# peterbudai/redux

Measured on AMD Instinct MI355X. Metric: encode MB/s (whole node), per-block bitstream bit-exact, higher is better.
Workload: dtype u32

## Files before the change

### redux_amd/csrc/redux_hip.hip

```cpp
#include "redux_coder.hpp"
#include "redux_any.hpp"
#include "redux_gen.hpp"
#include "redux_encode.hpp"
#include "redux_decode.hpp"
#include "redux_decode_adaptive.hpp"
#include "redux_decode_wave.hpp"
#include "redux_decode_cells.hpp"
#include "redux_pack.hpp"
#include "redux_table.hpp"
#include "redux_coop.hpp"
#include "redux_synth.hpp"
#include "redux_static.hpp"
#include "redux_planes.hpp"
#include "redux_delta.hpp"
#include "redux_hist.hpp"
#include "redux_plane_static.hpp"
#include "redux_segment_static.hpp"
#include "redux_crc.hpp"
#include "redux_store.hpp"

#include "../../include/redux_hip.h"

#include <hip/hip_runtime.h>
#include <algorithm>
// ... 64 lines not shown
    a.out_sizes[blk] = (uint32_t)bo;
    a.status[blk]    = st;
    if (a.in_used)
        a.in_used[blk] = bi;
}

static inline uint64_t align_up(uint64_t v, uint64_t a) { return (v + a - 1) / a * a; }

struct Geometry {
    uint64_t nblocks;
    uint64_t slot_bytes;
    uint32_t slot_cap;
    uint32_t rc_n;
    uint32_t nfreeze;
    bool     u16, fixup;
    bool     any;
    bool     gen;
    uint64_t tree_bytes;
    bool     coop;
    bool     coop_linear;
    uint32_t pair_width;
    uint32_t coop_win;
    uint32_t coop_nwin;
    uint64_t off_rc, off_sizes, off_mode, off_slots, off_trees, off_table, off_seen, off_cstate, off_pairs, total;
};

static int check_params(const redux_params *p)
{
    if (!p)
        return REDUX_INVALID_INPUT;
    const int st = redux_params_check(p->symbol_bits, p->freq_bits, p->code_bits);
    if (st != REDUX_OK)
        return st;
    if (p->symbol_bits > 16)
        return REDUX_UNSUPPORTED;
    return REDUX_OK;
}

static bool is_any(const redux_params *p) { return p->symbol_bits != 8 || p->code_bits > 32; }
static uint64_t gen_updates(const redux_params *p, uint32_t block_size)
{
    const uint64_t nsym    = (uint64_t)block_size * 8 / p->symbol_bits;
    const uint64_t nfreeze = ((1ull << p->freq_bits) - 1) - ((1ull << p->symbol_bits) + 1);
    return nsym < nfreeze ? nsym : nfreeze;
}
static bool gen_decode_cells(const redux_params *p, uint32_t block_size)
// ... 49 lines not shown
    const bool     freezes  = 257ull + n > freq_max;
    const uint64_t bits     = freezes ? n * (p->freq_bits + 2) : n * 9;
    return bits / 8 + 1024;
}

static Geometry geometry(const redux_params *p, uint64_t in_len, uint32_t block_size, bool static_model = false, bool allow_coop = true)
{
    Geometry g;
    memset(&g, 0, sizeof g);
    g.nblocks = in_len == 0 ? 1 : (in_len + block_size - 1) / block_size;
    const uint64_t cap = static_model ? ((uint64_t)block_size + 1) * (p->freq_bits + 2) / 8 + 1024 : slot_cap_for(p, block_size);
    g.slot_cap   = cap > 0xFFFFFF00ull ? 0xFFFFFF00u : (uint32_t)cap;
    g.slot_bytes = align_up((uint64_t)g.slot_cap + 32, 128);
    if (((g.slot_bytes / 128) & 1) == 0)
        g.slot_bytes += 128;
    const uint64_t freq_max = (1ull << p->freq_bits) - 1;
    g.nfreeze = (uint32_t)(freq_max - 257);
    const uint64_t maxlen = in_len < block_size ? in_len : block_size;
    g.rc_n  = (uint32_t)((maxlen < g.nfreeze ? maxlen : g.nfreeze) + 1);
    g.u16   = block_size <= 65536;
    g.fixup = (257ull + (uint64_t)(g.rc_n - 1)) >= (1ull << 17);
    g.rc_n += 32;
    g.any = !static_model && is_any(p);
    if (static_model)
        g.rc_n = 0;
    g.gen = !static_model && is_gen(p, block_size) && 64ull * g.slot_bytes < (1ull << 32);
    if (g.gen) {
        const uint64_t k0      = (1ull << p->symbol_bits) + 1;
        const uint64_t nsym    = maxlen * 8 / p->symbol_bits;
        const uint64_t nfreeze = freq_max - k0;
        g.any     = false;
        g.nfreeze = (uint32_t)(nfreeze < 0xFFFFFFFFull ? nfreeze : 0xFFFFFFFFull);
        g.rc_n    = (uint32_t)((nsym < nfreeze ? nsym : nfreeze) + 1 + 32);
        g.u16     = false;
        g.fixup   = true;
        g.tree_bytes = 0;
    }
    if (g.any) {
        g.rc_n       = 0;
        g.u16        = false;
        g.fixup      = true;
        g.tree_bytes = align_up(((1ull << p->symbol_bits) + 2) * 4, 256);
    }
    g.pair_width = g.u16 ? 64u : 1u;
    const uint64_t lanes_total = g.u16 ? (g.nblocks + 63) / 64 * 64 : g.nblocks;
    g.coop_win  = block_size + 1;
// ... 72 lines not shown

static EncKernel pick_encode_kernel(const Geometry &g, const redux_params *p, bool aligned16, uint32_t block_size)
{
    if (g.gen)
        return p->symbol_bits < 8 ? EncKernel::Gen : EncKernel::GenPair;
    if (g.any)
        return EncKernel::Any;
    bool coop = g.coop;
#ifdef REDUX_AB
    if (getenv("REDUX_ENCODE_KERNEL"))
        coop = false;
#endif
    if (coop)
        return p->code_bits == 32 ? EncKernel::CoopCb32 : EncKernel::Coop;
    bool pair = g.u16 && aligned16 && encode_lanes(g, block_size) == 64;
#ifdef REDUX_AB
    const char *force = getenv("REDUX_ENCODE_KERNEL");
    if (force && !strcmp(force, "single"))
        pair = false;
#endif
    if (pair)
        return p->code_bits == 32 ? EncKernel::PairCb32 : EncKernel::Pair;
    return g.u16 ? EncKernel::SingleU16 : EncKernel::SingleU32;
}

static DecKernel pick_decode_kernel(const Geometry &g, const redux_params *p, uint64_t nslots = 0, uint32_t block_size = 0, bool table = false)
{
    if (g.gen) {
        if (gen_needs_fixup(p, block_size))
            return DecKernel::CellsFixup;
        return gen_decode_in_workspace(p, nslots ? nslots : ~0ull) ? DecKernel::CellsWorkspace : DecKernel::Cells;
    }
    if (g.any)
        return DecKernel::Any;
    if (cells8_takes(p, block_size, nslots, table))
        return cells8_needs_fixup(p, block_size) ? DecKernel::Cells8Fixup : DecKernel::Cells8;
    bool wave = nslots != 0 && nslots <= kWaveDecMaxBlocks && !(g.u16 && !g.fixup);
#ifdef REDUX_AB
    if (getenv("REDUX_DECODE_KERNEL"))
        wave = false;
#endif
    if (wave)
        return g.fixup ? DecKernel::WaveFixup : DecKernel::Wave;
    bool lock = g.u16 && !g.fixup;
#ifdef REDUX_AB
    if (getenv("REDUX_DECODE_KERNEL"))
// ... 282 lines not shown
{
    if (check_params(p) != REDUX_OK || block_size == 0)
        return 0;
    return geometry(p, block_size, block_size).slot_cap;
}

uint64_t redux_encode_bound(const redux_params *p, uint64_t in_len, uint32_t block_size)
{
    if (check_params(p) != REDUX_OK || block_size == 0)
        return 0;
    const Geometry g = geometry(p, in_len, block_size);
    return g.nblocks * (uint64_t)g.slot_cap;
}

uint64_t redux_encode_workspace_bytes(const redux_params *p, uint64_t in_len, uint32_t block_size)
{
    if (check_params(p) != REDUX_OK || block_size == 0)
        return 0;
    return geometry(p, in_len, block_size).total;
}

static int encode_slots_impl(const redux_params *p, const void *d_in, uint64_t in_len, uint32_t block_size,
                             const redux_block *d_table, uint64_t tbl_blocks, bool tbl_aligned16, void *d_block_status,
                             void *d_workspace, uint64_t workspace_bytes, void *stream, uint64_t nblocks_real = 0)
{
    int st = check_params(p);
    if (st != REDUX_OK)
        return st;
    if (block_size == 0 || !d_workspace || !d_block_status || (in_len && !d_in))
        return REDUX_INVALID_INPUT;
    const Geometry g = geometry_ws(p, d_table ? tbl_blocks * (uint64_t)block_size : in_len, block_size, workspace_bytes);
    if (d_table && (g.gen || g.any || in_len > 0xFFFFFFFFull || tbl_blocks == 0))
        return tbl_blocks == 0 ? REDUX_INVALID_INPUT : REDUX_UNSUPPORTED;
    if (workspace_bytes < g.total)
        return REDUX_OUTPUT_TOO_SMALL;
    if (((uintptr_t)d_workspace) & 255)
        return REDUX_INVALID_INPUT;
    hipStream_t s  = (hipStream_t)stream;
    uint8_t    *ws = (uint8_t *)d_workspace;

    if (d_table) {
        TableCheckArgs ta;
        ta.in         = d_table;
        ta.out        = (redux_block *)(ws + g.off_table);
        ta.nentries   = tbl_blocks;
        ta.nblocks    = nblocks_real;
        ta.bytes      = in_len;
        ta.block_size = block_size;
// ... 58 lines not shown
    k_fill_rc<<<(g.rc_n + 255) / 256, 256, 0, s>>>((double *)(ws + g.off_rc), g.rc_n);

    EncArgs a;
    a.in         = (const uint8_t *)d_in;
    a.in_len     = in_len;
    a.nblocks    = g.nblocks;
    a.slots      = ws + g.off_slots;
    a.slot_bytes = g.slot_bytes;
    a.sizes      = (uint32_t *)(ws + g.off_sizes);
    a.status     = (int32_t *)d_block_status;
    a.rc         = (const double *)(ws + g.off_rc);
    a.block_size = block_size;
    a.slot_cap   = g.slot_cap;
    a.nfreeze    = g.nfreeze;
    a.code_bits  = p->code_bits;
    a.aligned16  = ((((uintptr_t)d_in) & 15) == 0 && (d_table ? tbl_aligned16 : (block_size & 15) == 0)) ? 1 : 0;
    a.claims     = (uint32_t *)(ws + g.off_mode + 256);
    a.table      = d_table;
    a.pair_width = g.pair_width;
    a.win0 = 0; a.winlen = block_size + 1; a.rc_frozen = 0.0; a.cstate = nullptr; a.cbase = nullptr;
    a.lanes = encode_lanes(g, block_size);
    const uint32_t grid = (uint32_t)((g.nblocks + a.lanes - 1) / a.lanes);
    const EncKernel which = pick_encode_kernel(g, p, a.aligned16 != 0, block_size);
    if (which == EncKernel::PairCb32 || which == EncKernel::Pair || which == EncKernel::CoopCb32 || which == EncKernel::Coop)
        HIP_TRY(hipMemsetAsync(ws + g.off_mode, g.coop_linear ? 2 : (1 | 2), 4, s));
    switch (which) {
    case EncKernel::CoopCb32:
    case EncKernel::Coop: {
        uint2         *pairs = (uint2 *)(ws + g.off_pairs);
        const uint32_t cgrid = (uint32_t)((g.nblocks + 63) / 64);
        const bool     cb32  = which == EncKernel::CoopCb32;
        {
            const double r = 1.0 / (double)(257ull + g.nfreeze);
            uint64_t     u;
            memcpy(&u, &r, 8);
            u += 4;
            memcpy(&a.rc_frozen, &u, 8);
        }
        a.winlen = g.coop_win;
        a.cstate = !g.u16 ? (uint32_t *)(ws + g.off_cstate) : nullptr;
        a.cbase  = a.cstate ? a.cstate + g.nblocks * 8 : nullptr;
        if (g.u16) {
            k_coop_model<false><<<(uint32_t)g.nblocks, 64, 0, s>>>(a, pairs);
            if (g.fixup) {
                if (cb32) k_coop_chain<true, true><<<cgrid, 128, 0, s>>>(a, pairs);
                else      k_coop_chain<false, true><<<cgrid, 128, 0, s>>>(a, pairs);
// ... 34 lines not shown
            }
#undef REDUX_COOP_LAUNCH
        }
        break;
    }
    case EncKernel::PairCb32: k_encode_pair<false, true><<<grid, 128, 0, s>>>(a); break;
    case EncKernel::Pair: k_encode_pair<false, false><<<grid, 128, 0, s>>>(a); break;
    case EncKernel::SingleU16: k_encode<true, false><<<grid, 64, 0, s>>>(a); break;
    case EncKernel::SingleU32: k_encode<false, true><<<grid, 64, 0, s>>>(a); break;
    case EncKernel::Gen:
    case EncKernel::GenPair:
    case EncKernel::Any: break;
    }
    HIP_TRY(hipGetLastError());
    return REDUX_OK;
}

int redux_encode_slots_dev(const redux_params *p, const void *d_in, uint64_t in_len, uint32_t block_size,
                           void *d_block_status, void *d_workspace, uint64_t workspace_bytes, void *stream)
{
    return encode_slots_impl(p, d_in, in_len, block_size, nullptr, 0, false, d_block_status, d_workspace, workspace_bytes, stream);
}

static int compact_with(const Geometry &g, void *d_out, uint64_t out_cap, void *d_out_offsets, void *d_block_status,
                        void *d_summary, void *d_workspace, uint64_t workspace_bytes, void *stream,
                        const redux_block *d_table = nullptr, uint64_t nblocks_real = 0, const uint8_t *d_stored = nullptr,
                        const void *d_raw = nullptr, uint32_t block_size = 0)
{
    if (!d_workspace || !d_block_status || !d_out_offsets || !d_out)
        return REDUX_INVALID_INPUT;
    if (workspace_bytes < g.off_pairs)
        return REDUX_OUTPUT_TOO_SMALL;
    hipStream_t s  = (hipStream_t)stream;
    uint8_t    *ws = (uint8_t *)d_workspace;

    ScanArgs sa;
    sa.sizes   = (const uint32_t *)(ws + g.off_sizes);
    sa.status  = (const int32_t *)d_block_status;
    sa.offsets = (uint64_t *)d_out_offsets;
    sa.summary = (int32_t *)d_summary;
    sa.nblocks = d_table ? nblocks_real : g.nblocks;
    if (scan_is_coalesced(sa))
        k_scan_sizes_coalesced<<<1, 1024, 0, s>>>(sa);
    else
        k_scan_sizes<<<1, 1024, 0, s>>>(sa);

    CompactArgs ca;
    ca.slots      = ws + g.off_slots;
    ca.slot_bytes = g.slot_bytes;
    ca.offsets    = (const uint64_t *)d_out_offsets;
    ca.out        = (uint8_t *)d_out;
    ca.out_cap    = out_cap;
    ca.status     = (int32_t *)d_block_status;
    ca.summary    = (int32_t *)d_summary;
    ca.nblocks    = g.nblocks;
    ca.mode       = (const uint32_t *)(ws + g.off_mode);
    ca.cap_rows   = (uint32_t)(g.slot_bytes / 4);
    ca.table      = d_table;
    ca.stored     = d_stored;
    ca.raw        = (const uint8_t *)d_raw;
    ca.block_size = block_size;
    k_compact<<<(uint32_t)g.nblocks, 256, 0, s>>>(ca);
    if (!g.any && !g.gen && (g.u16 || g.coop)) {
        const uint32_t tiles = (ca.cap_rows + kTileRows - 1) / kTileRows + 1;
        const uint32_t groups = (uint32_t)((g.nblocks + 63) / 64);
        k_compact_rows<<<(groups + 7) / 8 * 8 * tiles, 256, 0, s>>>(ca);
    }
    HIP_TRY(hipGetLastError());
    return REDUX_OK;
}

int redux_compact_slots_dev(const redux_params *p, uint64_t in_len, uint32_t block_size, void *d_out,
                            uint64_t out_cap, void *d_out_offsets, void *d_block_status, void *d_summary,
                            void *d_workspace, uint64_t workspace_bytes, void *stream)
{
    int st = check_params(p);
    if (st != REDUX_OK)
        return st;
    if (block_size == 0)
        return REDUX_INVALID_INPUT;
    return compact_with(geometry_ws(p, in_len, block_size, workspace_bytes), d_out, out_cap, d_out_offsets, d_block_status, d_summary,
                        d_workspace, workspace_bytes, stream);
}

int redux_encode_blocks_dev(const redux_params *p, const void *d_in, uint64_t in_len, uint32_t block_size,
                            void *d_out, uint64_t out_cap, void *d_out_offsets, void *d_block_status,
                            void *d_summary, void *d_workspace, uint64_t workspace_bytes, void *stream)
{
    int st = redux_encode_slots_dev(p, d_in, in_len, block_size, d_block_status, d_workspace, workspace_bytes, stream);
    if (st != REDUX_OK)
        return st;
    return redux_compact_slots_dev(p, in_len, block_size, d_out, out_cap, d_out_offsets, d_block_status, d_summary,
                                   d_workspace, workspace_bytes, stream);
}

int redux_encode_blocks_v_dev(const redux_params *p, const void *d_in, uint64_t in_bytes, const void *d_table,
                              uint64_t nentries, uint64_t nblocks, uint32_t block_size, uint32_t flags, void *d_out,
                              uint64_t out_cap, void *d_out_offsets, void *d_block_status, void *d_summary, void *d_workspace,
                              uint64_t workspace_bytes, void *stream)
{
    if (!d_table || nblocks == 0 || nentries < nblocks)
        return REDUX_INVALID_INPUT;
    if (nentries > 0xFFFFFFF0ull || nblocks > 0xFFFFFFF0ull || !d_block_status || !d_workspace)
        return REDUX_INVALID_INPUT;
    int st = encode_slots_impl(p, d_in, in_bytes, block_size, (const redux_block *)d_table, nentries,
                               (flags & REDUX_V_ALIGNED16) != 0, d_block_status, d_workspace, workspace_bytes, stream, nblocks);
    if (st != REDUX_OK)
        return st;
    const Geometry g = geometry_ws(p, nentries * (uint64_t)block_size, block_size, workspace_bytes);
    st = compact_with(g, d_out, out_cap, d_out_offsets, d_block_status, d_summary, d_workspace, workspace_bytes, stream,
                      (const redux_block *)((uint8_t *)d_workspace + g.off_table), nblocks);
    if (st != REDUX_OK)
        return st;
    k_table_verdict<<<1, 1, 0, (hipStream_t)stream>>>((const uint32_t *)((uint8_t *)d_workspace + g.off_seen) + table_seen_words(nblocks) - 1,
                                                      (int32_t *)d_summary);
    HIP_TRY(hipGetLastError());
    return REDUX_OK;
}

uint64_t redux_block_count_v(const uint64_t *in_len, uint64_t ninputs, uint32_t block_size)
{
    if (block_size == 0 || (ninputs && !in_len))
        return 0;
    uint64_t n = 0;
    for (uint64_t i = 0; i < ninputs; i++)
        n += redux_block_count(in_len[i], block_size);
    return n;
}

uint64_t redux_block_table_v(const uint64_t *in_off, const uint64_t *in_len, uint64_t ninputs, uint32_t block_size,
                             redux_block *table)
{
    const uint64_t nb = redux_block_count_v(in_len, ninputs, block_size);
// ... 559 lines not shown
    HIP_TRY(hipMemsetAsync(ws + g.off_mode, 0, 256, s));
    StaticEncArgs a;
    a.in         = (const uint8_t *)d_in;
    a.in_len     = in_len;
    a.nblocks    = g.nblocks;
    a.slots      = ws + g.off_slots;
    a.slot_bytes = g.slot_bytes;
    a.sizes      = (uint32_t *)(ws + g.off_sizes);
    a.status     = (int32_t *)d_block_status;
    a.rc         = static_rc(cum[kStaticEntries - 1]);
    a.block_size = block_size;
    a.slot_cap   = g.slot_cap;
    a.code_bits  = p->code_bits;
    a.aligned16  = ((((uintptr_t)d_in) & 15) == 0 && (block_size & 15) == 0) ? 1 : 0;
    memcpy(a.tab.cum, cum, sizeof a.tab.cum);
    const uint32_t grid = (uint32_t)((g.nblocks + 63) / 64);
    switch (pick_static_encode_kernel(p, cum[kStaticEntries - 1], g.nblocks)) {
    case StaticEncKernel::Fixup: k_encode_static<true, false><<<grid, 64, 0, s>>>(a); break;
    case StaticEncKernel::Cb32Solo: k_encode_static<false, true, true><<<grid, 64, 0, s>>>(a); break;
    case StaticEncKernel::Cb32: k_encode_static<false, true><<<grid, 64, 0, s>>>(a); break;
    case StaticEncKernel::Narrow: k_encode_static<false, false><<<grid, 64, 0, s>>>(a); break;
    }
    HIP_TRY(hipGetLastError());
    return compact_with(g, d_out, out_cap, d_out_offsets, d_block_status, d_summary, d_workspace, workspace_bytes, stream);
}

int redux_static_decode_blocks_dev(const redux_params *p, const uint32_t *cum, const void *d_in,
                                   const void *d_in_offsets, uint64_t nblocks, uint32_t block_size, void *d_out,
                                   uint64_t out_cap, void *d_out_sizes, void *d_block_status, void *d_summary,
                                   void *stream)
{
    int st = static_check(p, cum);
    if (st != REDUX_OK)
        return st;
    if (block_size == 0 || !d_in_offsets || !d_out_sizes || !d_block_status)
        return REDUX_INVALID_INPUT;
    if (nblocks == 0)
        return REDUX_OK;
    if (out_cap < nblocks * (uint64_t)block_size)
        return REDUX_OUTPUT_TOO_SMALL;
    hipStream_t   s = (hipStream_t)stream;
    StaticDecArgs a;
    a.in         = (const uint8_t *)d_in;
    a.in_offsets = (const uint64_t *)d_in_offsets;
    a.nblocks    = nblocks;
    a.out        = (uint8_t *)d_out;
    a.out_sizes  = (uint32_t *)d_out_sizes;
// ... 624 lines not shown
    a.c.nblocks    = g.nblocks;
    a.c.slots      = ws + g.off_slots;
    a.c.slot_bytes = g.slot_bytes;
    a.c.sizes      = (uint32_t *)(ws + g.off_sizes);
    a.c.status     = (int32_t *)d_block_status;
    a.c.rc         = static_rc(total);
    a.c.block_size = block_size;
    a.c.slot_cap   = g.slot_cap;
    a.c.code_bits  = p->code_bits;
    a.c.aligned16  = ((((uintptr_t)d_x) & 15) == 0 && (block_size & 15) == 0) ? 1 : 0;
    a.t.cum        = (const uint32_t *)d_cum;
    a.t.E          = E;
    a.t.total      = total;
    a.t.rc257      = static_rc(kStaticEntries - 1);
    const uint64_t slots = plane_slots(g.nblocks, E);
    const uint32_t grid  = (uint32_t)(slots * E);
    switch (pick_static_encode_kernel(p, total, 64 * E * slots)) {
    case StaticEncKernel::Fixup: k_encode_plane_static<true, false><<<grid, 64, 0, s>>>(a); break;
    case StaticEncKernel::Cb32Solo: k_encode_plane_static<false, true, true><<<grid, 64, 0, s>>>(a); break;
    case StaticEncKernel::Cb32: k_encode_plane_static<false, true><<<grid, 64, 0, s>>>(a); break;
    case StaticEncKernel::Narrow: k_encode_plane_static<false, false><<<grid, 64, 0, s>>>(a); break;
    }
    HIP_TRY(hipGetLastError());
    return compact_with(g, d_out, out_cap, d_out_offsets, d_block_status, d_summary, d_workspace, workspace_bytes, stream);
}

int redux_plane_static_encode_dev(const redux_params *p, const void *d_cum, uint32_t total, const void *d_in, uint64_t in_len,
                                  uint32_t block_size, uint32_t element_size, void *d_out, uint64_t out_cap, void *d_out_offsets,
                                  void *d_block_status, void *d_summary, void *d_workspace, uint64_t workspace_bytes, void *stream)
{
    int st = plane_static_check(p, element_size, total);
    if (st != REDUX_OK)
        return st;
    if (block_size == 0 || !d_cum || (!d_in && in_len) || !d_block_status || !d_workspace || (((uintptr_t)d_workspace) & 255))
        return REDUX_INVALID_INPUT;
    if (element_size == 1)
        return plane_static_encode_x(p, d_cum, total, d_in, in_len, block_size, 1, d_out, out_cap, d_out_offsets, d_block_status,
                                     d_summary, d_workspace, workspace_bytes, stream);
    const uint64_t copy = planes_copy_bytes(in_len);
    if (workspace_bytes < copy)
        return REDUX_OUTPUT_TOO_SMALL;
    uint8_t *x = (uint8_t *)d_workspace;
    if ((st = redux_planes_dev(d_in, x, in_len, block_size, element_size, 0, stream)) != REDUX_OK)
        return st;
    return plane_static_encode_x(p, d_cum, total, x, in_len, block_size, element_size, d_out, out_cap, d_out_offsets, d_block_status,
                                 d_summary, x + copy, workspace_bytes - copy, stream);
}
// ... 370 lines not shown
    a.c.slots      = ws + g.off_slots;
    a.c.slot_bytes = g.slot_bytes;
    a.c.sizes      = (uint32_t *)(ws + g.off_sizes);
    a.c.status     = (int32_t *)d_block_status;
    a.c.rc         = static_rc(total);
    a.c.block_size = block_size;
    a.c.slot_cap   = g.slot_cap;
    a.c.code_bits  = p->code_bits;
    a.c.aligned16  = ((((uintptr_t)d_x) & 15) == 0 && (block_size & 15) == 0) ? 1 : 0;
    a.t.p.cum      = (const uint32_t *)d_cum;
    a.t.p.E        = E;
    a.t.p.total    = total;
    a.t.p.rc257    = static_rc(kStaticEntries - 1);
    a.t.k          = G / (64 * E);
    const uint64_t slots = plane_slots(g.nblocks, E);
    const uint32_t grid  = (uint32_t)(slots * E);
    switch (pick_static_encode_kernel(p, total, 64 * E * slots)) {
    case StaticEncKernel::Fixup: k_encode_segment_static<true, false><<<grid, 64, 0, s>>>(a); break;
    case StaticEncKernel::Cb32Solo: k_encode_segment_static<false, true, true><<<grid, 64, 0, s>>>(a); break;
    case StaticEncKernel::Cb32: k_encode_segment_static<false, true><<<grid, 64, 0, s>>>(a); break;
    case StaticEncKernel::Narrow: k_encode_segment_static<false, false><<<grid, 64, 0, s>>>(a); break;
    }
    HIP_TRY(hipGetLastError());
    return compact_with(g, d_out, out_cap, d_out_offsets, d_block_status, d_summary, d_workspace, workspace_bytes, stream);
}

int redux_segment_static_encode_dev(const redux_params *p, const void *d_cum, uint32_t total, const void *d_in, uint64_t in_len,
                                    uint32_t block_size, uint32_t element_size, uint32_t segment_blocks, void *d_out, uint64_t out_cap,
                                    void *d_out_offsets, void *d_block_status, void *d_summary, void *d_workspace,
                                    uint64_t workspace_bytes, void *stream)
{
    int st = segment_static_check(p, element_size, segment_blocks, total);
    if (st != REDUX_OK)
        return st;
    if (block_size == 0 || !d_cum || (!d_in && in_len) || !d_block_status || !d_workspace || (((uintptr_t)d_workspace) & 255))
        return REDUX_INVALID_INPUT;
    if (element_size == 1)
        return segment_static_encode_x(p, d_cum, total, d_in, in_len, block_size, 1, segment_blocks, d_out, out_cap, d_out_offsets,
                                       d_block_status, d_summary, d_workspace, workspace_bytes, stream);
    const uint64_t copy = planes_copy_bytes(in_len);
    if (workspace_bytes < copy)
        return REDUX_OUTPUT_TOO_SMALL;
    uint8_t *x = (uint8_t *)d_workspace;
    if ((st = redux_planes_dev(d_in, x, in_len, block_size, element_size, 0, stream)) != REDUX_OK)
        return st;
    return segment_static_encode_x(p, d_cum, total, x, in_len, block_size, element_size, segment_blocks, d_out, out_cap, d_out_offsets,
                                   d_block_status, d_summary, x + copy, workspace_bytes - copy, stream);
// ... 195 lines not shown
}

int redux_encode_stored_dev(const redux_params *p, const void *d_in, uint64_t in_len, uint32_t block_size, uint32_t element_size,
                            uint32_t store_ratio, void *d_out, uint64_t out_cap, void *d_out_offsets, void *d_stored,
                            void *d_block_status, void *d_summary, void *d_workspace, uint64_t workspace_bytes, void *stream)
{
    int st = stored_check(p, block_size, element_size);
    if (st != REDUX_OK)
        return st;
    if (store_ratio > kStoreRatioOne || !d_workspace || !d_stored || !d_block_status || (in_len && !d_in))
        return REDUX_INVALID_INPUT;
    hipStream_t    s    = (hipStream_t)stream;
    const uint64_t copy = element_size > 1 ? planes_copy_bytes(in_len) : 0;
    if (workspace_bytes < copy)
        return REDUX_OUTPUT_TOO_SMALL;
    const void    *x    = d_in;
    if (element_size > 1) {
        if ((st = redux_planes_dev(d_in, d_workspace, in_len, block_size, element_size, 0, stream)) != REDUX_OK)
            return st;
        x = d_workspace;
    }
    uint8_t       *ws  = (uint8_t *)d_workspace + copy;
    const uint64_t wsb = workspace_bytes - copy;
    if ((st = encode_slots_impl(p, x, in_len, block_size, nullptr, 0, false, d_block_status, ws, wsb, stream)) != REDUX_OK)
        return st;
    const Geometry  g = geometry_ws(p, in_len, block_size, wsb);
    StoreSelectArgs sa;
    sa.status     = (const int32_t *)d_block_status;
    sa.sizes      = (uint32_t *)(ws + g.off_sizes);
    sa.stored     = (uint8_t *)d_stored;
    sa.nblocks    = g.nblocks;
    sa.in_len     = in_len;
    sa.block_size = block_size;
    sa.ratio      = store_ratio;
    const uint64_t wgs = (g.nblocks + 255) / 256;
    k_store_select<<<(uint32_t)(wgs < 1024 ? wgs : 1024), 256, 0, s>>>(sa);
    HIP_TRY(hipGetLastError());
    return compact_with(g, d_out, out_cap, d_out_offsets, d_block_status, d_summary, ws, wsb, stream, nullptr, 0,
                        (const uint8_t *)d_stored, x, block_size);
}

int redux_decode_stored_dev(const redux_params *p, const void *d_in, const void *d_in_offsets, const void *d_stored,
                            uint64_t out_len, uint32_t block_size, uint32_t element_size, void *d_out, uint64_t out_cap,
                            void *d_out_sizes, void *d_block_status, void *d_summary, void *d_workspace, uint64_t workspace_bytes,
                            void *stream)
{
    int st = stored_check(p, block_size, element_size);
    if (st != REDUX_OK)
        return st;
    if (!d_workspace || !d_in_offsets || !d_stored || !d_out_sizes || !d_block_status || (out_len && !d_out))
        return REDUX_INVALID_INPUT;
    if (out_cap < out_len || workspace_bytes < redux_decode_stored_workspace_bytes(p, out_len, block_size, element_size))
        return REDUX_OUTPUT_TOO_SMALL;
    if (((uintptr_t)d_workspace) & 255)
        return REDUX_INVALID_INPUT;
    hipStream_t    s       = (hipStream_t)stream;
    const uint64_t nblocks = redux_block_count(out_len, block_size);
    const uint64_t copy    = element_size > 1 ? planes_copy_bytes(nblocks * (uint64_t)block_size) : 0;
    uint8_t       *t       = element_size > 1 ? (uint8_t *)d_workspace : (uint8_t *)d_out;
    redux_block   *table   = (redux_block *)((uint8_t *)d_workspace + copy);
    uint8_t       *dws     = (uint8_t *)table + store_table_bytes(nblocks);
// ... 202 lines not shown
```

### redux_amd/csrc/redux_pack.hpp

```cpp
#pragma once

#include "redux_coder.hpp"
#include "redux_encode.hpp"
#include "redux_store.hpp"

#include "../../include/redux_hip.h"

#include <hip/hip_runtime.h>
#include <stdint.h>

namespace redux {

__global__ void k_summarize(const int32_t *status, uint64_t nblocks, int32_t *summary)
{
    uint32_t bad = 0;
    uint64_t first = ~0ull;
    for (uint64_t b = (uint64_t)blockIdx.x * blockDim.x + threadIdx.x; b < nblocks; b += (uint64_t)gridDim.x * blockDim.x)
        if (status[b] != REDUX_OK) {
            bad++;
            if (first == ~0ull)
                first = b;
        }
    if (bad) {
        atomicAdd(&summary[1], (int32_t)bad);
// ... 187 lines not shown
    if (tid == 0 && a.summary) {
        a.summary[0] = bad_cnt ? (int32_t)(bad_first & 0xFF) : REDUX_OK;
        a.summary[1] = (int32_t)bad_cnt;
    }
}

struct CompactArgs {
    const uint8_t  *slots;
    uint64_t        slot_bytes;
    const uint64_t *offsets;
    uint8_t        *out;
    uint64_t        out_cap;
    int32_t        *status;
    int32_t        *summary;
    uint64_t        nblocks;
    const uint32_t *mode;
    uint32_t        cap_rows;
    const redux_block *table;
    const uint8_t  *stored;
    const uint8_t  *raw;
    uint32_t        block_size;
};

__global__ void __launch_bounds__(256) k_compact(CompactArgs a)
{
    const uint64_t b = blockIdx.x;
    const uint32_t mode = *a.mode;
    if (b >= a.nblocks || ((mode & 1u) && !a.stored))
        return;
    const uint32_t bx  = (mode & 2u) ? 3u : 0u;
    const uint32_t sel = (mode & 2u) ? 0x00010203u : 0x03020100u;
    const uint64_t lb = a.table ? a.table[b].index : b;
    if (lb == kIdleEntry)
        return;
    const bool raw = a.stored && a.stored[lb];
    if ((mode & 1u) && !raw)
        return;
    const uint64_t o0 = a.offsets[lb], o1 = a.offsets[lb + 1];
    const uint32_t tid = threadIdx.x;
    if (o1 > a.out_cap) {
        if (tid == 0) {
            if (a.status[lb] == REDUX_OK)
                a.status[lb] = REDUX_OUTPUT_TOO_SMALL;
            if (a.summary) {
                atomicCAS(&a.summary[0], REDUX_OK, REDUX_OUTPUT_TOO_SMALL);
                atomicAdd(&a.summary[1], 1);
            }
        }
        return;
    }
    const uint32_t n   = (uint32_t)(o1 - o0);
    const uint8_t *src = a.slots + b * a.slot_bytes;
    uint8_t       *dst = a.out + o0;
    if (raw) {
        store_copy(a.raw + lb * a.block_size, dst, n, tid, 256);
        return;
    }

    uint32_t head = (uint32_t)((16 - ((uintptr_t)dst & 15)) & 15);
    if (head > n)
        head = n;
    if (tid < head)
// ... 1 lines not shown
    const uint32_t nchunks = (n - head) >> 4;
    const uint32_t dq = head >> 2, r = head & 3;
    const uint4   *s16 = reinterpret_cast<const uint4 *>(src);
    uint4         *d16 = reinterpret_cast<uint4 *>(dst + head);
    for (uint32_t i = tid; i < nchunks; i += 256) {
        const uint4    A = s16[i], B = s16[i + 1];
        const uint32_t d[8] = {A.x, A.y, A.z, A.w, B.x, B.y, B.z, B.w};
        uint32_t       v[5];
#pragma unroll
        for (int k = 0; k < 5; k++)
            v[k] = __builtin_amdgcn_perm(0u, dq == 0 ? d[k] : dq == 1 ? d[k + 1] : dq == 2 ? d[k + 2] : d[k + 3], sel);
        uint4 o;
        o.x = __builtin_amdgcn_alignbyte(v[1], v[0], r);
        o.y = __builtin_amdgcn_alignbyte(v[2], v[1], r);
        o.z = __builtin_amdgcn_alignbyte(v[3], v[2], r);
        o.w = __builtin_amdgcn_alignbyte(v[4], v[3], r);
        d16[i] = o;
    }
    const uint32_t done = head + (nchunks << 4);
    if (tid < n - done)
        dst[done + tid] = src[(done + tid) ^ bx];
}

constexpr uint32_t kTileRows = 64;
__global__ void __launch_bounds__(256) k_compact_rows(CompactArgs a)
{
    const uint32_t mode = *a.mode;
    if ((mode & 1u) == 0)
        return;
    const uint32_t sel = (mode & 2u) ? 0x00010203u : 0x03020100u;
    __shared__ uint32_t tile[(kTileRows + 1) * 65];
    __shared__ uint64_t s_dst[64];
    __shared__ uint32_t s_n[64], s_sh[64];
    __shared__ uint32_t s_maxj;
    const uint32_t tiles = (a.cap_rows + kTileRows - 1) / kTileRows + 1;
    const uint32_t y   = blockIdx.x >> 3;
    const uint64_t g   = (uint64_t)(y / tiles) * 8 + (blockIdx.x & 7u);
    const uint32_t r0  = (y % tiles) * kTileRows;
    if (g * 64 >= a.nblocks)
        return;
    const uint32_t tid   = threadIdx.x;
    if (tid == 0)
        s_maxj = 0;
    __syncthreads();
    if (tid < 64) {
        const uint64_t b = g * 64 + tid;
        uint64_t       d = 0;
        uint32_t       n = 0, sh = 0;
        const uint64_t lb = b < a.nblocks ? (a.table ? a.table[b].index : b) : kIdleEntry;
        if (lb != kIdleEntry && !(a.stored && a.stored[lb])) {
            const uint64_t o0 = a.offsets[lb], o1 = a.offsets[lb + 1];
            if (o1 <= a.out_cap) {
                n  = (uint32_t)(o1 - o0);
                sh = (uint32_t)((uintptr_t)(a.out + o0) & 3);
                d  = (uint64_t)(uintptr_t)(a.out + o0) - sh;
                atomicMax(&s_maxj, (sh + n + 3) >> 2);
            } else if (r0 == 0) {
                if (a.status[lb] == REDUX_OK)
                    a.status[lb] = REDUX_OUTPUT_TOO_SMALL;
                if (a.summary) {
                    atomicCAS(&a.summary[0], REDUX_OK, REDUX_OUTPUT_TOO_SMALL);
                    atomicAdd(&a.summary[1], 1);
                }
            }
        }
        s_dst[tid] = d;
        s_n[tid]   = n;
        s_sh[tid]  = sh;
    }
    __syncthreads();
    if (r0 >= s_maxj)
        return;
    const uint4 *area = reinterpret_cast<const uint4 *>(a.slots + g * (64 * a.slot_bytes + 128));
    uint4 v[4], lead = make_uint4(0, 0, 0, 0);
#pragma unroll
    for (int q = 0; q < 4; q++) {
        const uint32_t e = tid + 256 * q, r = r0 + (e >> 4);
        v[q] = r < a.cap_rows ? area[(uint64_t)r * 16 + (e & 15)] : make_uint4(0, 0, 0, 0);
    }
    if (tid < 16 && r0 > 0)
        lead = area[(uint64_t)(r0 - 1) * 16 + tid];
#pragma unroll
    for (int q = 0; q < 4; q++) {
        const uint32_t e = tid + 256 * q;
        uint32_t      *w = &tile[((e >> 4) + 1) * 65 + (e & 15) * 4];
        w[0] = v[q].x; w[1] = v[q].y; w[2] = v[q].z; w[3] = v[q].w;
    }
    if (tid < 16) {
        uint32_t *w = &tile[tid * 4];
        w[0] = lead.x; w[1] = lead.y; w[2] = lead.z; w[3] = lead.w;
    }
    __syncthreads();
    const uint32_t wave = tid >> 6, t = tid & 63;
#pragma unroll 2
    for (uint32_t it = 0; it < 4; it++) {
        const uint32_t l  = wave * 16 + it * 4 + (t >> 4);
        const uint32_t jq = (t & 15) * 4;
        const uint64_t d  = s_dst[l];
        const uint32_t n = s_n[l], sh = s_sh[l];
        const uint32_t j0 = r0 + jq;
        if (d == 0 || j0 >= ((sh + n + 3) >> 2))
            continue;
        uint32_t src[5];
#pragma unroll
        for (int c = 0; c < 5; c++)
            src[c] = __builtin_amdgcn_perm(0u, tile[(jq + c) * 65 + l], sel);
        uint32_t w[4];
#pragma unroll
        for (int c = 0; c < 4; c++)
            w[c] = sh ? __builtin_amdgcn_alignbyte(src[c + 1], src[c], 4 - sh) : src[c + 1];
        uint8_t      *A     = reinterpret_cast<uint8_t *>((uintptr_t)d) + 4 * (uint64_t)j0;
        const int64_t first = (int64_t)4 * j0 - sh;
        if (first >= 0 && first + 16 <= (int64_t)n) {
            typedef uint32_t u32x4 __attribute__((ext_vector_type(4), aligned(4)));
            *reinterpret_cast<u32x4 *>(A) = u32x4{w[0], w[1], w[2], w[3]};
        } else {
#pragma unroll
            for (int c = 0; c < 4; c++) {
                const int64_t f = first + 4 * c;
                if (f >= 0 && f + 4 <= (int64_t)n) {
                    *reinterpret_cast<uint32_t *>(A + 4 * c) = w[c];
                } else {
                    for (int i = 0; i < 4; i++)
                        if (f + i >= 0 && f + i < (int64_t)n)
                            A[4 * c + i] = (uint8_t)(w[c] >> (8 * i));
                }
            }
        }
    }
}

}
```

Before: 364,800.

## Make row-compaction persistent with register-prefetched tiles and skip the unused compaction kernel

```diff
diff --git a/redux_amd/csrc/redux_hip.hip b/redux_amd/csrc/redux_hip.hip
--- a/redux_amd/csrc/redux_hip.hip
+++ b/redux_amd/csrc/redux_hip.hip
@@ -110,6 +110,7 @@
     uint32_t pair_width;
     uint32_t coop_win;
     uint32_t coop_nwin;
+    bool     static_model;
     uint64_t off_rc, off_sizes, off_mode, off_slots, off_trees, off_table, off_seen, off_cstate, off_pairs, total;
 };
 
@@ -205,6 +206,7 @@
     g.fixup = (257ull + (uint64_t)(g.rc_n - 1)) >= (1ull << 17);
     g.rc_n += 32;
     g.any = !static_model && is_any(p);
+    g.static_model = static_model;
     if (static_model)
         g.rc_n = 0;
     g.gen = !static_model && is_gen(p, block_size) && 64ull * g.slot_bytes < (1ull << 32);
@@ -323,6 +325,50 @@
     if (pair)
         return p->code_bits == 32 ? EncKernel::PairCb32 : EncKernel::Pair;
     return g.u16 ? EncKernel::SingleU16 : EncKernel::SingleU32;
+}
+
+enum class SlotLayout { Linear, Rows, Either };
+
+static SlotLayout slot_layout_of(EncKernel which, const Geometry &g)
+{
+    switch (which) {
+    case EncKernel::PairCb32:
+    case EncKernel::Pair: return SlotLayout::Rows;
+    case EncKernel::CoopCb32:
+    case EncKernel::Coop: return g.coop_linear ? SlotLayout::Linear : SlotLayout::Rows;
+    default: return SlotLayout::Linear;
+    }
+}
+
+static SlotLayout slot_layout(const Geometry &g, uint32_t block_size)
+{
+    if (g.static_model || g.gen || g.any)
+        return SlotLayout::Linear;
+#ifdef REDUX_AB
+    if (getenv("REDUX_ENCODE_KERNEL"))
+        return SlotLayout::Either;
+#endif
+    if (g.coop)
+        return g.coop_linear ? SlotLayout::Linear : SlotLayout::Rows;
+    if (!g.u16 || encode_lanes(g, block_size) != 64)
+        return SlotLayout::Linear;
+    if (block_size & 15)
+        return SlotLayout::Linear;
+    return SlotLayout::Either;
+}
+
+constexpr uint32_t kCompactRows = 128, kCompactOversub = 2;
+
+template <uint32_t ROWS>
+static void launch_compact_rows(const CompactArgs &ca, uint32_t oversub, bool linear, hipStream_t s)
+{
+    const uint32_t per_cu   = std::min<uint32_t>(8u, (160u << 10) / compact_rows_lds_bytes<ROWS>());
+    const uint32_t resident = cu_count() * per_cu;
+    const uint32_t groups8  = (uint32_t)((ca.nblocks + 63) / 64 + 7) / 8 * 8;
+    const uint32_t tiles    = (ca.cap_rows + ROWS - 1) / ROWS + 1;
+    uint32_t splits = (oversub * resident + groups8 - 1) / groups8;
+    splits = std::max<uint32_t>(1u, std::min<uint32_t>(splits, tiles / kRowsMinTiles));
+    k_compact_rows<ROWS><<<groups8 * splits, 256, 0, s>>>(ca, splits, linear ? 1u : 0u);
 }
 
 static DecKernel pick_decode_kernel(const Geometry &g, const redux_params *p, uint64_t nslots = 0, uint32_t block_size = 0, bool table = false)
@@ -651,8 +697,11 @@
 
 static int encode_slots_impl(const redux_params *p, const void *d_in, uint64_t in_len, uint32_t block_size,
                              const redux_block *d_table, uint64_t tbl_blocks, bool tbl_aligned16, void *d_block_status,
-                             void *d_workspace, uint64_t workspace_bytes, void *stream, uint64_t nblocks_real = 0)
-{
+                             void *d_workspace, uint64_t workspace_bytes, void *stream, uint64_t nblocks_real = 0,
+                             SlotLayout *left = nullptr)
+{
+    if (left)
+        *left = SlotLayout::Linear;
     int st = check_params(p);
     if (st != REDUX_OK)
         return st;
@@ -757,6 +806,8 @@
     a.lanes = encode_lanes(g, block_size);
     const uint32_t grid = (uint32_t)((g.nblocks + a.lanes - 1) / a.lanes);
     const EncKernel which = pick_encode_kernel(g, p, a.aligned16 != 0, block_size);
+    if (left)
+        *left = slot_layout_of(which, g);
     if (which == EncKernel::PairCb32 || which == EncKernel::Pair || which == EncKernel::CoopCb32 || which == EncKernel::Coop)
         HIP_TRY(hipMemsetAsync(ws + g.off_mode, g.coop_linear ? 2 : (1 | 2), 4, s));
     switch (which) {
@@ -837,7 +888,7 @@
     return encode_slots_impl(p, d_in, in_len, block_size, nullptr, 0, false, d_block_status, d_workspace, workspace_bytes, stream);
 }
 
-static int compact_with(const Geometry &g, void *d_out, uint64_t out_cap, void *d_out_offsets, void *d_block_status,
+static int compact_with(const Geometry &g, SlotLayout left, void *d_out, uint64_t out_cap, void *d_out_offsets, void *d_block_status,
                         void *d_summary, void *d_workspace, uint64_t workspace_bytes, void *stream,
                         const redux_block *d_table = nullptr, uint64_t nblocks_real = 0, const uint8_t *d_stored = nullptr,
                         const void *d_raw = nullptr, uint32_t block_size = 0)
@@ -875,11 +926,24 @@
     ca.stored     = d_stored;
     ca.raw        = (const uint8_t *)d_raw;
     ca.block_size = block_size;
-    k_compact<<<(uint32_t)g.nblocks, 256, 0, s>>>(ca);
-    if (!g.any && !g.gen && (g.u16 || g.coop)) {
-        const uint32_t tiles = (ca.cap_rows + kTileRows - 1) / kTileRows + 1;
-        const uint32_t groups = (uint32_t)((g.nblocks + 63) / 64);
-        k_compact_rows<<<(groups + 7) / 8 * 8 * tiles, 256, 0, s>>>(ca);
+    const bool linear_kernel = left == SlotLayout::Linear || d_stored != nullptr;
+    if (linear_kernel)
+        k_compact<<<(uint32_t)g.nblocks, 256, 0, s>>>(ca);
+    if (left != SlotLayout::Linear) {
+        uint32_t rows = kCompactRows, oversub = kCompactOversub;
+#ifdef REDUX_AB
+        if (getenv("REDUX_COMPACT_ROWS"))
+            rows = (uint32_t)atoi(getenv("REDUX_COMPACT_ROWS"));
+        if (getenv("REDUX_COMPACT_OVERSUB"))
+            oversub = (uint32_t)atoi(getenv("REDUX_COMPACT_OVERSUB"));
+        if (rows == 64)
+            launch_compact_rows<64>(ca, oversub, !linear_kernel, s);
+        else if (rows == 256)
+            launch_compact_rows<256>(ca, oversub, !linear_kernel, s);
+        else
+#endif
+        launch_compact_rows<128>(ca, oversub, !linear_kernel, s);
+        (void)rows;
     }
     HIP_TRY(hipGetLastError());
     return REDUX_OK;
@@ -894,19 +958,21 @@
         return st;
     if (block_size == 0)
         return REDUX_INVALID_INPUT;
-    return compact_with(geometry_ws(p, in_len, block_size, workspace_bytes), d_out, out_cap, d_out_offsets, d_block_status, d_summary,
-                        d_workspace, workspace_bytes, stream);
+    const Geometry g = geometry_ws(p, in_len, block_size, workspace_bytes);
+    return compact_with(g, slot_layout(g, block_size), d_out, out_cap, d_out_offsets, d_block_status, d_summary, d_workspace,
+                        workspace_bytes, stream);
 }
 
 int redux_encode_blocks_dev(const redux_params *p, const void *d_in, uint64_t in_len, uint32_t block_size,
                             void *d_out, uint64_t out_cap, void *d_out_offsets, void *d_block_status,
                             void *d_summary, void *d_workspace, uint64_t workspace_bytes, void *stream)
 {
-    int st = redux_encode_slots_dev(p, d_in, in_len, block_size, d_block_status, d_workspace, workspace_bytes, stream);
-    if (st != REDUX_OK)
-        return st;
-    return redux_compact_slots_dev(p, in_len, block_size, d_out, out_cap, d_out_offsets, d_block_status, d_summary,
-                                   d_workspace, workspace_bytes, stream);
+    SlotLayout left;
+    int st = encode_slots_impl(p, d_in, in_len, block_size, nullptr, 0, false, d_block_status, d_workspace, workspace_bytes, stream, 0, &left);
+    if (st != REDUX_OK)
+        return st;
+    return compact_with(geometry_ws(p, in_len, block_size, workspace_bytes), left, d_out, out_cap, d_out_offsets, d_block_status,
+                        d_summary, d_workspace, workspace_bytes, stream);
 }
 
 int redux_encode_blocks_v_dev(const redux_params *p, const void *d_in, uint64_t in_bytes, const void *d_table,
@@ -918,12 +984,13 @@
         return REDUX_INVALID_INPUT;
     if (nentries > 0xFFFFFFF0ull || nblocks > 0xFFFFFFF0ull || !d_block_status || !d_workspace)
         return REDUX_INVALID_INPUT;
+    SlotLayout left;
     int st = encode_slots_impl(p, d_in, in_bytes, block_size, (const redux_block *)d_table, nentries,
-                               (flags & REDUX_V_ALIGNED16) != 0, d_block_status, d_workspace, workspace_bytes, stream, nblocks);
+                               (flags & REDUX_V_ALIGNED16) != 0, d_block_status, d_workspace, workspace_bytes, stream, nblocks, &left);
     if (st != REDUX_OK)
         return st;
     const Geometry g = geometry_ws(p, nentries * (uint64_t)block_size, block_size, workspace_bytes);
-    st = compact_with(g, d_out, out_cap, d_out_offsets, d_block_status, d_summary, d_workspace, workspace_bytes, stream,
+    st = compact_with(g, left, d_out, out_cap, d_out_offsets, d_block_status, d_summary, d_workspace, workspace_bytes, stream,
                       (const redux_block *)((uint8_t *)d_workspace + g.off_table), nblocks);
     if (st != REDUX_OK)
         return st;
@@ -1529,7 +1596,7 @@
     case StaticEncKernel::Narrow: k_encode_static<false, false><<<grid, 64, 0, s>>>(a); break;
     }
     HIP_TRY(hipGetLastError());
-    return compact_with(g, d_out, out_cap, d_out_offsets, d_block_status, d_summary, d_workspace, workspace_bytes, stream);
+    return compact_with(g, SlotLayout::Linear, d_out, out_cap, d_out_offsets, d_block_status, d_summary, d_workspace, workspace_bytes, stream);
 }
 
 int redux_static_decode_blocks_dev(const redux_params *p, const uint32_t *cum, const void *d_in,
@@ -2200,7 +2267,7 @@
     case StaticEncKernel::Narrow: k_encode_plane_static<false, false><<<grid, 64, 0, s>>>(a); break;
     }
     HIP_TRY(hipGetLastError());
-    return compact_with(g, d_out, out_cap, d_out_offsets, d_block_status, d_summary, d_workspace, workspace_bytes, stream);
+    return compact_with(g, SlotLayout::Linear, d_out, out_cap, d_out_offsets, d_block_status, d_summary, d_workspace, workspace_bytes, stream);
 }
 
 int redux_plane_static_encode_dev(const redux_params *p, const void *d_cum, uint32_t total, const void *d_in, uint64_t in_len,
@@ -2617,7 +2684,7 @@
     case StaticEncKernel::Narrow: k_encode_segment_static<false, false><<<grid, 64, 0, s>>>(a); break;
     }
     HIP_TRY(hipGetLastError());
-    return compact_with(g, d_out, out_cap, d_out_offsets, d_block_status, d_summary, d_workspace, workspace_bytes, stream);
+    return compact_with(g, SlotLayout::Linear, d_out, out_cap, d_out_offsets, d_block_status, d_summary, d_workspace, workspace_bytes, stream);
 }
 
 int redux_segment_static_encode_dev(const redux_params *p, const void *d_cum, uint32_t total, const void *d_in, uint64_t in_len,
@@ -2859,7 +2926,8 @@
     }
     uint8_t       *ws  = (uint8_t *)d_workspace + copy;
     const uint64_t wsb = workspace_bytes - copy;
-    if ((st = encode_slots_impl(p, x, in_len, block_size, nullptr, 0, false, d_block_status, ws, wsb, stream)) != REDUX_OK)
+    SlotLayout left;
+    if ((st = encode_slots_impl(p, x, in_len, block_size, nullptr, 0, false, d_block_status, ws, wsb, stream, 0, &left)) != REDUX_OK)
         return st;
     const Geometry  g = geometry_ws(p, in_len, block_size, wsb);
     StoreSelectArgs sa;
@@ -2873,7 +2941,7 @@
     const uint64_t wgs = (g.nblocks + 255) / 256;
     k_store_select<<<(uint32_t)(wgs < 1024 ? wgs : 1024), 256, 0, s>>>(sa);
     HIP_TRY(hipGetLastError());
-    return compact_with(g, d_out, out_cap, d_out_offsets, d_block_status, d_summary, ws, wsb, stream, nullptr, 0,
+    return compact_with(g, left, d_out, out_cap, d_out_offsets, d_block_status, d_summary, ws, wsb, stream, nullptr, 0,
                         (const uint8_t *)d_stored, x, block_size);
 }
 
diff --git a/redux_amd/csrc/redux_pack.hpp b/redux_amd/csrc/redux_pack.hpp
--- a/redux_amd/csrc/redux_pack.hpp
+++ b/redux_amd/csrc/redux_pack.hpp
@@ -233,12 +233,8 @@
     uint32_t        block_size;
 };
 
-__global__ void __launch_bounds__(256) k_compact(CompactArgs a)
-{
-    const uint64_t b = blockIdx.x;
-    const uint32_t mode = *a.mode;
-    if (b >= a.nblocks || ((mode & 1u) && !a.stored))
-        return;
+__device__ __forceinline__ void compact_linear(const CompactArgs &a, uint64_t b, uint32_t mode, uint32_t tid)
+{
     const uint32_t bx  = (mode & 2u) ? 3u : 0u;
     const uint32_t sel = (mode & 2u) ? 0x00010203u : 0x03020100u;
     const uint64_t lb = a.table ? a.table[b].index : b;
@@ -248,7 +244,6 @@
     if ((mode & 1u) && !raw)
         return;
     const uint64_t o0 = a.offsets[lb], o1 = a.offsets[lb + 1];
-    const uint32_t tid = threadIdx.x;
     if (o1 > a.out_cap) {
         if (tid == 0) {
             if (a.status[lb] == REDUX_OK)
@@ -296,24 +291,40 @@
         dst[done + tid] = src[(done + tid) ^ bx];
 }
 
-constexpr uint32_t kTileRows = 64;
-__global__ void __launch_bounds__(256) k_compact_rows(CompactArgs a)
-{
+__global__ void __launch_bounds__(256) k_compact(CompactArgs a)
+{
+    const uint64_t b = blockIdx.x;
     const uint32_t mode = *a.mode;
-    if ((mode & 1u) == 0)
-        return;
+    if (b >= a.nblocks || ((mode & 1u) && !a.stored))
+        return;
+    compact_linear(a, b, mode, threadIdx.x);
+}
+
+constexpr uint32_t kRowsMinTiles = 4;
+template <uint32_t ROWS> constexpr uint32_t compact_rows_lds_bytes() { return ((ROWS + 1) * 65 + 64 * 4 + 2) * 4; }
+
+template <uint32_t ROWS>
+__global__ void __launch_bounds__(256) k_compact_rows(CompactArgs a, uint32_t splits, uint32_t linear)
+{
+    static_assert(ROWS % 64 == 0, "a wave stores 64-dword pieces of four streams at a time");
+    const uint32_t mode = *a.mode;
+    const uint32_t tid  = threadIdx.x;
+    if ((mode & 1u) == 0) {
+        if (linear)
+            for (uint64_t b = blockIdx.x; b < a.nblocks; b += gridDim.x)
+                compact_linear(a, b, mode, tid);
+        return;
+    }
     const uint32_t sel = (mode & 2u) ? 0x00010203u : 0x03020100u;
-    __shared__ uint32_t tile[(kTileRows + 1) * 65];
+    __shared__ uint32_t tile[(ROWS + 1) * 65];
     __shared__ uint64_t s_dst[64];
     __shared__ uint32_t s_n[64], s_sh[64];
     __shared__ uint32_t s_maxj;
-    const uint32_t tiles = (a.cap_rows + kTileRows - 1) / kTileRows + 1;
-    const uint32_t y   = blockIdx.x >> 3;
-    const uint64_t g   = (uint64_t)(y / tiles) * 8 + (blockIdx.x & 7u);
-    const uint32_t r0  = (y % tiles) * kTileRows;
+    const uint32_t y  = blockIdx.x >> 3;
+    const uint64_t g  = (uint64_t)(y / splits) * 8 + (blockIdx.x & 7u);
+    const uint32_t sp = y % splits;
     if (g * 64 >= a.nblocks)
         return;
-    const uint32_t tid   = threadIdx.x;
     if (tid == 0)
         s_maxj = 0;
     __syncthreads();
@@ -329,7 +340,7 @@
                 sh = (uint32_t)((uintptr_t)(a.out + o0) & 3);
                 d  = (uint64_t)(uintptr_t)(a.out + o0) - sh;
                 atomicMax(&s_maxj, (sh + n + 3) >> 2);
-            } else if (r0 == 0) {
+            } else if (sp == 0) {
                 if (a.status[lb] == REDUX_OK)
                     a.status[lb] = REDUX_OUTPUT_TOO_SMALL;
                 if (a.summary) {
@@ -343,65 +354,80 @@
         s_sh[tid]  = sh;
     }
     __syncthreads();
-    if (r0 >= s_maxj)
-        return;
-    const uint4 *area = reinterpret_cast<const uint4 *>(a.slots + g * (64 * a.slot_bytes + 128));
-    uint4 v[4], lead = make_uint4(0, 0, 0, 0);
-#pragma unroll
-    for (int q = 0; q < 4; q++) {
-        const uint32_t e = tid + 256 * q, r = r0 + (e >> 4);
-        v[q] = r < a.cap_rows ? area[(uint64_t)r * 16 + (e & 15)] : make_uint4(0, 0, 0, 0);
-    }
-    if (tid < 16 && r0 > 0)
-        lead = area[(uint64_t)(r0 - 1) * 16 + tid];
-#pragma unroll
-    for (int q = 0; q < 4; q++) {
-        const uint32_t e = tid + 256 * q;
-        uint32_t      *w = &tile[((e >> 4) + 1) * 65 + (e & 15) * 4];
-        w[0] = v[q].x; w[1] = v[q].y; w[2] = v[q].z; w[3] = v[q].w;
-    }
-    if (tid < 16) {
-        uint32_t *w = &tile[tid * 4];
-        w[0] = lead.x; w[1] = lead.y; w[2] = lead.z; w[3] = lead.w;
-    }
-    __syncthreads();
+    const uint32_t maxj   = s_maxj;
+    const uint32_t ntiles = (maxj + ROWS - 1) / ROWS;
+    const uint32_t t0     = (uint32_t)((uint64_t)ntiles * sp / splits);
+    const uint32_t t1     = (uint32_t)((uint64_t)ntiles * (sp + 1) / splits);
+    if (t0 >= t1)
+        return;
+    const uint4   *area = reinterpret_cast<const uint4 *>(a.slots + g * (64 * a.slot_bytes + 128));
+    const uint32_t rlim = maxj < a.cap_rows ? maxj : a.cap_rows;
+    constexpr int  kQ   = ROWS / 16;
+    uint4 v[kQ], lead = make_uint4(0, 0, 0, 0);
+    auto  load_tile = [&](uint32_t r0) {
+#pragma unroll
+        for (int q = 0; q < kQ; q++) {
+            const uint32_t e = tid + 256 * q, r = r0 + (e >> 4);
+            v[q] = r < rlim ? area[(uint64_t)r * 16 + (e & 15)] : make_uint4(0, 0, 0, 0);
+        }
+        if (tid < 16 && r0 > 0)
+            lead = area[(uint64_t)(r0 - 1) * 16 + tid];
+    };
+    load_tile(t0 * ROWS);
     const uint32_t wave = tid >> 6, t = tid & 63;
+    for (uint32_t ti = t0; ti < t1; ti++) {
+        const uint32_t r0 = ti * ROWS;
+#pragma unroll
+        for (int q = 0; q < kQ; q++) {
+            const uint32_t e = tid + 256 * q;
+            uint32_t      *w = &tile[((e >> 4) + 1) * 65 + (e & 15) * 4];
+            w[0] = v[q].x; w[1] = v[q].y; w[2] = v[q].z; w[3] = v[q].w;
+        }
+        if (tid < 16) {
+            uint32_t *w = &tile[tid * 4];
+            w[0] = lead.x; w[1] = lead.y; w[2] = lead.z; w[3] = lead.w;
+        }
+        __syncthreads();
+        if (ti + 1 < t1)
+            load_tile(r0 + ROWS);
 #pragma unroll 2
-    for (uint32_t it = 0; it < 4; it++) {
-        const uint32_t l  = wave * 16 + it * 4 + (t >> 4);
-        const uint32_t jq = (t & 15) * 4;
-        const uint64_t d  = s_dst[l];
-        const uint32_t n = s_n[l], sh = s_sh[l];
-        const uint32_t j0 = r0 + jq;
-        if (d == 0 || j0 >= ((sh + n + 3) >> 2))
-            continue;
-        uint32_t src[5];
-#pragma unroll
-        for (int c = 0; c < 5; c++)
-            src[c] = __builtin_amdgcn_perm(0u, tile[(jq + c) * 65 + l], sel);
-        uint32_t w[4];
-#pragma unroll
-        for (int c = 0; c < 4; c++)
-            w[c] = sh ? __builtin_amdgcn_alignbyte(src[c + 1], src[c], 4 - sh) : src[c + 1];
-        uint8_t      *A     = reinterpret_cast<uint8_t *>((uintptr_t)d) + 4 * (uint64_t)j0;
-        const int64_t first = (int64_t)4 * j0 - sh;
-        if (first >= 0 && first + 16 <= (int64_t)n) {
-            typedef uint32_t u32x4 __attribute__((ext_vector_type(4), aligned(4)));
-            *reinterpret_cast<u32x4 *>(A) = u32x4{w[0], w[1], w[2], w[3]};
-        } else {
-#pragma unroll
-            for (int c = 0; c < 4; c++) {
-                const int64_t f = first + 4 * c;
-                if (f >= 0 && f + 4 <= (int64_t)n) {
-                    *reinterpret_cast<uint32_t *>(A + 4 * c) = w[c];
-                } else {
-                    for (int i = 0; i < 4; i++)
-                        if (f + i >= 0 && f + i < (int64_t)n)
-                            A[4 * c + i] = (uint8_t)(w[c] >> (8 * i));
+        for (uint32_t it = 0; it < (uint32_t)kQ; it++) {
+            const uint32_t l  = wave * 16 + (it / (ROWS / 64)) * 4 + (t >> 4);
+            const uint32_t jq = (it % (ROWS / 64)) * 64 + (t & 15) * 4;
+            const uint64_t d  = s_dst[l];
+            const uint32_t n = s_n[l], sh = s_sh[l];
+            const uint32_t j0 = r0 + jq;
+            if (d == 0 || j0 >= ((sh + n + 3) >> 2))
+                continue;
+            uint32_t src[5];
+#pragma unroll
+            for (int c = 0; c < 5; c++)
+                src[c] = __builtin_amdgcn_perm(0u, tile[(jq + c) * 65 + l], sel);
+            uint32_t w[4];
+#pragma unroll
+            for (int c = 0; c < 4; c++)
+                w[c] = sh ? __builtin_amdgcn_alignbyte(src[c + 1], src[c], 4 - sh) : src[c + 1];
+            uint8_t      *A     = reinterpret_cast<uint8_t *>((uintptr_t)d) + 4 * (uint64_t)j0;
+            const int64_t first = (int64_t)4 * j0 - sh;
+            if (first >= 0 && first + 16 <= (int64_t)n) {
+                typedef uint32_t u32x4 __attribute__((ext_vector_type(4), aligned(4)));
+                *reinterpret_cast<u32x4 *>(A) = u32x4{w[0], w[1], w[2], w[3]};
+            } else {
+#pragma unroll
+                for (int c = 0; c < 4; c++) {
+                    const int64_t f = first + 4 * c;
+                    if (f >= 0 && f + 4 <= (int64_t)n) {
+                        *reinterpret_cast<uint32_t *>(A + 4 * c) = w[c];
+                    } else {
+                        for (int i = 0; i < 4; i++)
+                            if (f + i >= 0 && f + i < (int64_t)n)
+                                A[4 * c + i] = (uint8_t)(w[c] >> (8 * i));
+                    }
                 }
             }
         }
-    }
-}
-
-}
+        __syncthreads();
+    }
+}
+
+}
```

Result: slower. 346,100 (-5.1%).
